# kspalaiologos/bzip3

Measured on AMD Instinct MI355X. Metric: MiB/s encode+decode round-trip, 8 MiB blocks, higher is better.
Workload: dtype u8

## Files before the change

bzip3_amd/__init__.py:

```python
import ctypes as C
import os

_HERE = os.path.dirname(os.path.abspath(__file__))
LIB_PATH = os.path.join(_HERE, "lib", "libbzip3.so")

BZ3_OK = 0
BZ3_ERR_OUT_OF_BOUNDS = -1
BZ3_ERR_BWT = -2
BZ3_ERR_CRC = -3
BZ3_ERR_MALFORMED_HEADER = -4
BZ3_ERR_TRUNCATED_DATA = -5
BZ3_ERR_DATA_TOO_BIG = -6
BZ3_ERR_INIT = -7
BZ3_ERR_DATA_SIZE_TOO_SMALL = -8

T_NAMES = ["crc", "rle", "lzp", "bwt", "cm", "copy", "_6", "_7"]

_lib = None


def _declare(L, strict=True):
    vp, i32, u32, sz = C.c_void_p, C.c_int32, C.c_uint32, C.c_size_t
    sig = {
        "bz3_version": (C.c_char_p, []),
# ... 23 lines not shown
        "bz3_hip_cm_variant_for": (C.c_int, [C.c_int, C.c_int, C.c_int]),
        "bz3_hip_set_lean_states": (C.c_int, [C.c_int]),
        "bz3_hip_release_cached_memory": (None, []),
        "bz3_hip_set_keep_workspace": (C.c_int, [C.c_int]),
        "bz3_hip_set_front_end_duo": (C.c_int, [C.c_int]),
        "bz3_hip_set_workspace_headroom": (None, [C.c_longlong]),
        "bz3_hip_workspace_headroom": (sz, []),
        "bz3_hip_debug_headroom_events": (C.c_uint, [C.c_int, C.POINTER(C.c_uint)]),
        "bz3_hip_debug_ring_contexts": (sz, [sz, sz, sz, sz, sz, sz, C.c_int, sz]),
        "bz3_hip_debug_arena_slack": (sz, [sz]),
        "bz3_hip_debug_cm_launches": (C.c_uint, [C.c_int]),
        "bz3_hip_debug_workspace_bytes": (sz, [sz, C.c_int]),
        "bz3_hip_debug_cached_bytes": (sz, [C.c_int]),
        "bz3_hip_encode_block_device": (i32, [vp, vp, i32]),
        "bz3_hip_decode_block_device": (i32, [vp, vp, sz, i32, i32]),
        "bz3_hip_encode_blocks_device": (None, [vp, vp, vp, i32]),
        "bz3_hip_decode_blocks_device": (None, [vp, vp, vp, vp, vp, i32]),
        "bz3_hip_compress_device": (C.c_int, [u32, vp, vp, sz, C.POINTER(sz)]),
        "bz3_hip_decompress_device": (C.c_int, [vp, vp, sz, C.POINTER(sz)]),
        "bz3_hip_frame_decoded_size_device": (C.c_int, [vp, sz, C.POINTER(sz)]),
        "bz3_hip_compress_device_many": (C.c_int, [u32, i32, C.POINTER(vp), C.POINTER(sz), C.POINTER(vp), C.POINTER(sz), C.POINTER(C.c_int)]),
        "bz3_hip_decompress_device_many": (C.c_int, [i32, C.POINTER(vp), C.POINTER(sz), C.POINTER(vp), C.POINTER(sz), C.POINTER(C.c_int)]),
        "bz3_hip_frame_decoded_sizes_device": (C.c_int, [i32, C.POINTER(vp), C.POINTER(sz), C.POINTER(sz), C.POINTER(C.c_int)]),
        "bz3_hip_debug_copy_segments": (i32, [vp, vp, C.POINTER(C.c_uint64), i32]),
        "bz3_hip_compress_device_planes": (C.c_int, [u32, u32, vp, vp, sz, C.POINTER(sz)]),
        "bz3_hip_decompress_device_planes": (C.c_int, [u32, vp, vp, sz, C.POINTER(sz)]),
        "bz3_hip_compress_device_planes_many": (C.c_int, [u32, i32, C.POINTER(u32), C.POINTER(vp), C.POINTER(sz), C.POINTER(vp), C.POINTER(sz), C.POINTER(C.c_int)]),
        "bz3_hip_decompress_device_planes_many": (C.c_int, [i32, C.POINTER(u32), C.POINTER(vp), C.POINTER(sz), C.POINTER(vp), C.POINTER(sz), C.POINTER(C.c_int)]),
        "bz3_hip_debug_planes": (i32, [vp, vp, C.POINTER(C.c_uint64), i32]),
        "bz3_hip_compress_device_delta": (C.c_int, [u32, u32, vp, vp, vp, sz, C.POINTER(sz)]),
        "bz3_hip_decompress_device_delta": (C.c_int, [u32, vp, vp, sz, vp, sz, C.POINTER(sz)]),
        "bz3_hip_compress_device_delta_many": (C.c_int, [u32, i32, C.POINTER(u32), C.POINTER(vp), C.POINTER(vp), C.POINTER(sz), C.POINTER(vp), C.POINTER(sz), C.POINTER(C.c_int)]),
        "bz3_hip_decompress_device_delta_many": (C.c_int, [i32, C.POINTER(u32), C.POINTER(vp), C.POINTER(sz), C.POINTER(vp), C.POINTER(sz), C.POINTER(vp), C.POINTER(sz), C.POINTER(C.c_int)]),
        "bz3_hip_crc32c_device": (C.c_int, [vp, sz, u32, C.POINTER(u32)]),
        "bz3_hip_crc32c_device_many": (C.c_int, [i32, C.POINTER(vp), C.POINTER(sz), C.POINTER(u32), C.POINTER(u32)]),
        "bz3_hip_debug_crc_launches": (C.c_uint, [C.c_int]),
        "bz3_hip_debug_delta": (i32, [vp, vp, vp, C.POINTER(C.c_uint64), i32]),
        "bz3_hip_decompress_device_range": (C.c_int, [u32, vp, sz, C.c_uint64, vp, sz, vp, C.POINTER(sz)]),
        "bz3_hip_decompress_device_range_many": (C.c_int, [i32, C.POINTER(u32), C.POINTER(vp), C.POINTER(sz), C.POINTER(C.c_uint64), C.POINTER(vp), C.POINTER(sz),
                                                           C.POINTER(vp), C.POINTER(sz), C.POINTER(C.c_int)]),
        "bz3_hip_debug_range": (i32, [vp, vp, vp, C.POINTER(C.c_uint64), i32]),
        "bz3_hip_last_timings": (None, [vp, C.POINTER(C.c_float)]),
        "bz3_hip_last_bwt_stats": (None, [vp, C.POINTER(i32), C.POINTER(i32), C.POINTER(C.c_uint64)]),
        "bz3_hip_stage_crc32c": (u32, [vp, sz, u32]),
        "bz3_hip_stage_mrle_encode": (i32, [vp, i32, vp]),
        "bz3_hip_stage_mrle_decode": (C.c_int, [vp, vp, i32, i32]),
        "bz3_hip_stage_lzp_encode": (i32, [vp, i32, vp]),
        "bz3_hip_stage_lzp_decode": (i32, [vp, i32, vp, i32]),
        "bz3_hip_stage_bwt": (i32, [vp, vp, i32]),
        "bz3_hip_stage_unbwt": (i32, [vp, vp, i32, i32]),
        "bz3_hip_stage_last_ms": (C.c_float, []),
        "bz3_hip_debug_sort_u32": (i32, [vp, u32, C.c_int, C.c_int, vp, vp]),
        "bz3_hip_debug_scan_u32": (i32, [vp, u32, vp]),
        "bz3_hip_debug_cu_masks": (i32, [C.c_int, C.c_int, vp, vp]),
        "bz3_hip_set_collect_window_us": (None, [C.c_int]),
        "bz3_hip_debug_collected_batches": (C.c_uint, [C.c_int, C.POINTER(C.c_uint)]),
        "bz3_hip_stage_cm_encode": (i32, [vp, i32, vp]),
        "bz3_hip_stage_cm_decode": (None, [vp, i32, vp, i32]),
        "bz3_hip_stage_cm_decode_many": (C.c_float, [vp, i32, vp, i32, i32, vp]),
        "bz3_hip_stage_cm_encode_many": (C.c_float, [vp, i32, vp, C.POINTER(i32), i32]),
        "bz3_hip_encode_stream": (C.c_int, [C.c_int, C.c_int, i32, i32]),
        "bz3_hip_decode_stream": (C.c_int, [C.c_int, C.c_int, i32]),
    }
    for name, (res, args) in sig.items():
        if not strict and not hasattr(L, name):
            continue
        fn = getattr(L, name)
        fn.restype = res
        fn.argtypes = args
    return L


EXPORTED_SYMBOLS = None


def _share_hip_runtime_with_torch():
    if os.environ.get("BZ3_HIP_SYSTEM_RUNTIME") == "1":
        return
    try:
        import importlib.util

        spec = importlib.util.find_spec("torch")
        if spec is None or not spec.origin:
            return
        cand = os.path.join(os.path.dirname(spec.origin), "lib", "libamdhip64.so")
        if os.path.exists(cand):
            C.CDLL(cand, mode=C.RTLD_GLOBAL)
    except Exception:
        pass


def load(path=None):
    global _lib
    if _lib is not None and path is None:
        return _lib
    if path is None:
        _share_hip_runtime_with_torch()
    p = path or LIB_PATH
    if not os.path.exists(p):
        raise RuntimeError(
            f"{p} is missing: the HIP extension has not been built (python -m bzip3_amd.build). "
            "bzip3_amd has no CPU or PyTorch fallback by design."
        )
    L = _declare(C.CDLL(p), strict=path is None)
    if path is None:
        _lib = L
# ... 844 lines not shown
```

bzip3_amd/csrc/api.hip:

```cpp
#include <atomic>
#include <chrono>
#include <condition_variable>
#include <cstdio>
#include <cstdlib>
#include <exception>
#include <mutex>
#include <new>
#include <stdexcept>
#include <thread>
#include <type_traits>
#include <vector>

#include "../../include/bz3_hip.h"
#include "frame.hpp"
#include "planes.hpp"
#include "prims.hpp"
#include "sort.hpp"
#include "stages.hpp"

using namespace bz3;

namespace {

constexpr s32 KiB65 = 65 * 1024;
// ... 3115 lines not shown
        bwt_inverse(d, (u32)n, (u32)idx, o, a, e.s);
        HIP_CHECK(hipStreamSynchronize(e.s));
        g_stage_ms.store(std::chrono::duration<float, std::milli>(std::chrono::steady_clock::now() - t0).count());
        e.down(out, o, (size_t)n);
        return 0;
    });
}

BZIP3_API int32_t bz3_hip_debug_cu_masks(int cus, int reserve, uint32_t * side, uint32_t * rest) {
    if (cus < 32 || cus > 1024 || reserve < 8 || !side || !rest) return -1;
    std::vector<uint32_t> a, b;
    DeviceCtx::cu_masks(cus, reserve, a, b);
    for (size_t k = 0; k < a.size(); k++) {
        side[k] = a[k];
        rest[k] = b[k];
    }
    return (int32_t)a.size();
}

BZIP3_API int32_t bz3_hip_debug_scan_u32(uint32_t * data, uint32_t n, uint32_t * total) {
    return stage_guard([&]() -> s32 {
        if (n == 0) return -1;
        StageEnv e;
        u32 * d = (u32 *)e.dev((size_t)n * 4 + 64, data, (size_t)n * 4);
        u32 * t = (u32 *)e.dev(64);
        Arena a = e.ctx->arena_for(scan_temp_words(n) * 4 + (1u << 20));
        exclusive_scan_u32(d, n, t, a, e.s);
        e.down(data, d, (size_t)n * 4);
        if (total) *total = e.word(t);
        return 0;
    });
}

BZIP3_API int32_t bz3_hip_debug_sort_u32(const uint32_t * keys, uint32_t n, int key_bits, int digit_bits, uint32_t * sorted_keys, uint32_t * sorted_index) {
    return stage_guard([&]() -> s32 {
        if ((digit_bits != 8 && digit_bits != 9) || key_bits < 1 || key_bits > 32 || n == 0) return -1;
        StageEnv e;
        u32 * k[2] = {(u32 *)e.dev((size_t)n * 4 + 64, keys, (size_t)n * 4), (u32 *)e.dev((size_t)n * 4 + 64)};
        u32 * v[2] = {(u32 *)e.dev((size_t)n * 4 + 64), (u32 *)e.dev((size_t)n * 4 + 64)};
        Arena a = e.ctx->arena_for(radix_temp_bytes(n, digit_bits) + (1u << 20));
        int cur = 0, passes = 0;
        for (int shift = 0; shift < key_bits; shift += digit_bits, passes++) {
            const u32 * vin = passes ? v[cur] : nullptr;
            if (digit_bits == 9) radix_pass_bits<u32, 9>(k[cur], k[cur ^ 1], vin, v[cur ^ 1], n, shift, 0xFFFFFFFFu, 0u, a, e.s);
            else radix_pass<u32>(k[cur], k[cur ^ 1], vin, v[cur ^ 1], n, shift, 0xFFFFFFFFu, 0u, a, e.s);
            cur ^= 1;
        }
        e.down(sorted_keys, k[cur], (size_t)n * 4);
        e.down(sorted_index, v[cur], (size_t)n * 4);
        return passes;
    });
}

extern "C++" template <class Job, class Launch>
void stage_cm_job(StageEnv & e, Job job, Launch && go) {
    const int variant = cm_variant_for(e.ctx, 1, std::is_same<Job, CmEncodeJob>::value);
    u32 * status = nullptr;
    if (cm_variant_has_rows(variant)) {
        job.spill = dev_addr(e.dev(CM_SPILL_BYTES));
        status = (u32 *)e.dev(64);
        HIP_CHECK(hipMemsetAsync(status, 0, 64, e.s));
        job.status = dev_addr(status);
        job.miss_base = cm_variant_is_test(variant) ? 64u : CM_MISS_BASE;
        job.miss_shift = cm_variant_is_test(variant) ? 3u : CM_MISS_SHIFT;
    }
    Job * d_job = (Job *)e.dev(sizeof job, &job, sizeof job);
    go(d_job, 1u, e.s, variant);
    if (cm_variant_has_rows(variant) && e.word(status) != 0u) {
        g_cm_given_up.fetch_add(1u);
        go(d_job, 1u, e.s, (int)CM_VARIANT_FULL);
    }
}

BZIP3_API int32_t bz3_hip_stage_cm_encode(const uint8_t * in, int32_t n, uint8_t * out) {
    return stage_guard([&]() -> s32 {
        StageEnv e;
        u8 * d = e.dev((size_t)n + 64, in, (size_t)n);
        u8 * o = e.dev(bz3_bound((size_t)n) + 64);
        u32 * w = (u32 *)e.dev(64);
        const char * dbg = getenv("BZ3_CM_DEBUG");
        CmEncodeJob job{dev_addr(d), dev_addr(o), dev_addr(w), (u32)n, dbg ? (u32)atoi(dbg) : 0u};
        const char * tg = getenv("BZ3_CM_TEST_GAP");
        u8 * side = nullptr;
        if (tg) {
            const size_t g = (size_t)atol(tg);
            const char * ts = getenv("BZ3_CM_TEST_SIDE");
            const size_t side_cap = ts ? (size_t)atol(ts) : CM_SIDE_BYTES;
            u8 * both = e.dev(g + (size_t)n + 64);
            HIP_CHECK(hipMemcpy(both + g, d, (size_t)n, hipMemcpyDeviceToDevice));
            side = e.dev(side_cap + 64);
            o = both;
            job.in = dev_addr(both + g);
            job.out = dev_addr(both);
            job.gap = (u32)g;
            job.side = dev_addr(side);
            job.side_cap = (u32)side_cap;
        }
        stage_cm_job(e, job, [](const CmEncodeJob * j, u32 nj, hipStream_t st, int variant) { cm_encode_batch(j, nj, st, variant); });
        const u32 coded = e.word(w), sw = e.word(w + 1);
        if (coded == 0xFFFFFFFFu) return -1;
        const u32 head = (tg && sw < coded) ? sw : coded;
        e.down(out, o, (size_t)head);
        if (head < coded) e.down(out + head, side, (size_t)(coded - head));
        return (s32)coded;
    });
}
// ... 123 lines not shown
```

bzip3_amd/csrc/bwt.hip:

```cpp
#include <atomic>
#include <vector>

#include "prims.hpp"
#include "sort.hpp"
#include "stages.hpp"

namespace bz3 {

constexpr int BW_BLOCK = 256;
constexpr u32 V_HEAD = 0x80000000u;
constexpr u32 V_MASK = 0x3FFFFFFFu;

__global__ void __launch_bounds__(256) k_bwt_outside(const u32 * __restrict__ hist, u32 keep, u32 * __restrict__ out) {
    __shared__ u32 h[256];
    __shared__ u32 red[256 / WAVE + 1];
    const u32 c = threadIdx.x;
    h[c] = hist[c];
    __syncthreads();
    const u32 mine = h[c];
    u32 rank = 0;
    for (u32 k = 0; k < 256u; k++) rank += (h[k] > mine || (h[k] == mine && k < c)) ? 1u : 0u;
    const u32 tot = block_sum<256>(rank >= keep ? mine : 0u, red);
    if (c == 0) *out = tot;
}
// ... 1232 lines not shown
                st_g[out] = rank[j];
                out++;
            }
        }
    }
    __syncthreads();
    for (u32 idx = threadIdx.x; idx < all; idx += BW_BLOCK) {
        vals_out[tile_off + idx] = st_v[idx];
        slots_out[tile_off + idx] = st_s[idx];
        grp_out[tile_off + idx] = st_g[idx];
    }
}

__global__ void __launch_bounds__(BW_BLOCK) k_bwt_doubling_keys_grp(const u32 * __restrict__ vals, const u32 * __restrict__ grp, const u32 * __restrict__ isa, u32 m,
                                                                   u32 n, u32 h, u64 * __restrict__ keys) {
    const u32 k = blockIdx.x * BW_BLOCK + threadIdx.x;
    if (k >= m) return;
    const u32 s = vals[k];
    const u64 j = (u64)s + h;
    const u32 lo = (j < n) ? isa[j] + h : (n - 1u - s);
    keys[k] = ((u64)grp[k] << 32) | lo;
}

constexpr int IS_ITEMS = 8;
__global__ void __launch_bounds__(BW_BLOCK) k_isa_scatter(const u32 * __restrict__ suf, const u32 * __restrict__ rank, u32 n, u32 tiles, u32 * __restrict__ isa) {
    const u32 per = (tiles + 7u) / 8u;
    const u32 tile = (blockIdx.x & 7u) * per + (blockIdx.x >> 3);
    if (tile >= tiles) return;
    const u64 base = (u64)tile * (BW_BLOCK * IS_ITEMS) + threadIdx.x;
    u32 x[IS_ITEMS], r[IS_ITEMS];
#pragma unroll
    for (int k = 0; k < IS_ITEMS; k++) {
        const u64 i = base + (u64)k * BW_BLOCK;
        x[k] = suf[i < n ? i : (u64)n - 1];
        r[k] = rank[i < n ? i : (u64)n - 1];
    }
#pragma unroll
    for (int k = 0; k < IS_ITEMS; k++)
        if (base + (u64)k * BW_BLOCK < n) isa[x[k] & V_MASK] = r[k];
}

static int bits_for(u64 x) {
    int b = 0;
    while (x) { b++; x >>= 1; }
    return b ? b : 1;
}

size_t bwt_workspace_bytes(u64 n) {
    return n * (16 + 8 + 1 + 11 + 4 + 8 + 4 + 4 + 4) + n / 8 + radix_temp_bytes(n) + scan_temp_words(n) * 4 + (1u << 20) + 16384 + VLC_WORK_BYTES;
}

template <typename K>
static int sort_iota(const K * kin, K * k0, K * k1, u32 * v0, u32 * v1, u64 n, int bit_lo, int bit_hi, Arena & tmp, hipStream_t s, BwtStats & st) {
    radix_pass<K>(kin, k1, (const u32 *)nullptr, v1, n, bit_lo, 0xFFFFFFFFu, 0u, tmp, s);
    int cur = 1;
    K * kk[2] = {k0, k1};
    u32 * vv[2] = {v0, v1};
    st.radix_passes++;
    for (int shift = bit_lo + 8; shift < bit_hi; shift += 8) {
        radix_pass<K>(kk[cur], kk[cur ^ 1], (const u32 *)vv[cur], vv[cur ^ 1], n, shift, 0xFFFFFFFFu, 0u, tmp, s);
        cur ^= 1;
        st.radix_passes++;
    }
    return cur;
}

struct BwtSwitches {
    bool trace;
    int big_rounds_default;
    std::atomic<int> big_rounds;
};
static BwtSwitches & bwt_switches() {
    static BwtSwitches sw{getenv("BZ3_BWT_TRACE") != nullptr, getenv("BZ3_BWT_BIG_ROUNDS") ? atoi(getenv("BZ3_BWT_BIG_ROUNDS")) : 1,
                          {getenv("BZ3_BWT_BIG_ROUNDS") ? atoi(getenv("BZ3_BWT_BIG_ROUNDS")) : 1}};
    return sw;
}
void bwt_set_big_rounds(int k) { bwt_switches().big_rounds.store(k < 0 ? bwt_switches().big_rounds_default : k); }
struct BwtGrids {
    u32 wide, tail;
};
static BwtGrids bwt_grids(u32 n) {
    static const BwtGrids forced = [] {
        BwtGrids g{0, 0};
        if (const char * e = getenv("BZ3_BWT_GRIDS")) (void)sscanf(e, "%u,%u", &g.wide, &g.tail);
        return g;
    }();
    if (forced.wide && forced.tail) return forced;
    const u32 tail = n / (64u * 4u), wide = n / (64u * 4u * 16u);
    return BwtGrids{wide < 8u ? 8u : wide, tail < 32u ? 32u : tail};
}

__global__ void k_bwt_set_word(u32 * p, u32 v) { *p = v; }

s32 bwt_forward(const u8 * d_in, u32 n, u8 * d_out, Arena & tmp, hipStream_t s, BwtStats * stats, u32 * d_idx, u32 * d_outside) {
    if (d_outside && n < 2) HIP_CHECK(hipMemsetAsync(d_outside, 0, 4, s));
    if (n == 0) {
        if (d_idx) launch(k_bwt_set_word, dim3(1), dim3(1), 0, s, d_idx, 0u);
        return 0;
    }
    if (n == 1) {
        HIP_CHECK(hipMemcpyAsync(d_out, d_in, 1, hipMemcpyDeviceToDevice, s));
        if (d_idx) {
            launch(k_bwt_set_word, dim3(1), dim3(1), 0, s, d_idx, 1u);
            return 0;
        }
        HIP_CHECK(hipStreamSynchronize(s));
        return 1;
    }
    if (n > V_MASK) throw HipError{hipErrorUnknown, "block too large for the suffix sorter", __FILE__, __LINE__};
    const size_t mk = tmp.mark();
    u64 * key[2] = {tmp.take<u64>(n), tmp.take<u64>(n)};
    u32 * val[2] = {tmp.take<u32>(n), tmp.take<u32>(n)};
    u8 * pb = tmp.take<u8>(n);
    const u32 tiles = (u32)(((u64)n + TR_S - 1) / TR_S);
    u32 * tile_last = tmp.take<u32>(tiles + 1);
    u32 * carry = tmp.take<u32>(tiles + 1);
    const u32 sp_groups = (tiles + SP_GROUP - 1) / SP_GROUP;
    u32 * group_max = tmp.take<u32>(sp_groups + 1);
    u32 * group_carry = tmp.take<u32>(sp_groups + 1);
    u8 * dirty = tmp.take<u8>(tiles + 2);
    u32 * hbits = tmp.take<u32>(((size_t)n + 63) / 64 * 2 + (size_t)TR_S / 32 + 8);
    u32 * d_words = tmp.take<u32>(16);
    u32 * d_vlc = tmp.take<u32>(256);
    u32 * d_hist = tmp.take<u32>(256);
    BwtStats st;

    auto grid = [](u64 m) { return dim3((u32)((m + BW_BLOCK - 1) / BW_BLOCK)); };

    HIP_CHECK(hipMemsetAsync(d_hist, 0, 256 * sizeof(u32), s));
    HIP_CHECK(hipMemsetAsync(d_words, 0, 16 * sizeof(u32), s));
    HIP_CHECK(hipMemsetAsync(d_words + 5, 0xFF, sizeof(u32), s));
    launch(k_bwt_sym_hist, grid(((u64)n + 63) / 64), dim3(BW_BLOCK), 0, s, d_in, n, d_hist);
    if (d_outside) launch(k_bwt_outside, dim3(1), dim3(256), 0, s, (const u32 *)d_hist, (u32)BWT_ROUTE_KEEP, d_outside);
    {
        const size_t vm = tmp.mark();
        vlc_build_device(d_hist, d_vlc, tmp, s);
        tmp.release(vm);
    }

    launch(k_bwt_vlc_keys, grid(((u64)n + 7) / 8), dim3(BW_BLOCK), 0, s, d_in, n, (const u32 *)d_vlc, key[0]);
    const int cur = sort_iota<u64>(key[0], key[0], key[1], val[0], val[1], n, 8, 64, tmp, s, st);
    st.sorted_elements += n;
    st.rounds++;
    u32 * V = val[cur];
    launch(k_bwt_heads, dim3(tiles), dim3(BW_BLOCK), 0, s, (const u64 *)key[cur], V, pb, n, tile_last, hbits, d_words);
    launch(k_bwt_spine_a, dim3(sp_groups), dim3(SP_BLOCK), 0, s, (const u32 *)tile_last, tiles, carry, group_max);
    launch(k_bwt_spine_b, dim3(1), dim3(1024), 0, s, (const u32 *)group_max, sp_groups, group_carry);

    const u32 big_cap = n / 4;
    char * scratch = reinterpret_cast<char *>(key[0]);
    (void)scratch;
    u32 * big_slot = reinterpret_cast<u32 *>(key[0]);
    u32 * big_hp = big_slot + big_cap;
    u32 * bord[2] = {big_hp + big_cap, big_hp + 2 * (size_t)big_cap};
    u32 * bgk[2] = {bord[1] + big_cap, bord[1] + 2 * (size_t)big_cap};
    u32 * gv = bgk[1] + big_cap;
    u32 * ghp = gv + big_cap;
    u64 * bkey0 = key[1];
    u64 * bkey[2] = {bkey0 + big_cap, bkey0 + 2 * (size_t)big_cap};
    u64 * gkey = bkey0 + 3 * (size_t)big_cap;
    u8 * gpb = reinterpret_cast<u8 *>(val[cur ^ 1]);
    const u32 tail_cap = n;
    u32 * tail_v = tmp.take<u32>(tail_cap);
    u32 * tail_slot = tmp.take<u32>(tail_cap);
    u16 * tail_d = tmp.take<u16>(tail_cap);
    u8 * tail_pb = tmp.take<u8>(tail_cap);
    const u32 mid_cap = n / 64 + 16;
    u32 * mid_slot = tmp.take<u32>(mid_cap);
    u16 * mid_size = tmp.take<u16>(mid_cap);
    u32 g = 7;
    bool deep = false;
    u32 h_words[16];
    const BwtGrids grids = bwt_grids(n);
    for (int pass = 0;; pass++) {
        launch(k_bwt_route, dim3((tiles + RT_WAVES - 1) / RT_WAVES), dim3(RT_WAVES * WAVE), 0, s, n, (const u32 *)V, (const u8 *)pb, (const u32 *)hbits,
               (const u32 *)carry, (const u32 *)group_carry, (const u8 *)(pass ? dirty : nullptr), big_slot, big_hp, big_cap, mid_slot, mid_size, mid_cap, tail_v, tail_slot,
               tail_d, tail_pb, tail_cap, d_words);
        launch(k_bwt_wide, dim3(grids.wide), dim3(WR_WAVES * WAVE), 0, s, d_in, n, V, pb, (const u32 *)d_vlc, (const u32 *)mid_slot, (const u16 *)mid_size, mid_cap, tail_v,
               tail_slot, tail_d, tail_pb, tail_cap, d_words, (u32)pass + 1u);
        launch(k_bwt_tail, dim3(grids.tail), dim3(WAVE), 0, s, d_in, n, V, pb, (const u32 *)d_vlc, (const u32 *)tail_v, (const u32 *)tail_slot, (const u16 *)tail_d,
               (const u8 *)tail_pb, d_words, (u32)pass + 1u);
        HIP_CHECK(hipMemcpyAsync(h_words, d_words, sizeof h_words, hipMemcpyDeviceToHost, s));
        HIP_CHECK(hipStreamSynchronize(s));
        const u32 nb = h_words[0];
        if (bwt_switches().trace) fprintf(stderr, "[bwt] n %u pass %d depth %u: %u suffixes in groups > %d, %u groups through the wide kernel, %u suffixes through the tail kernel, %u given up, overflow %u\n", n, pass, g, nb, TR_G, h_words[8], h_words[4], h_words[1], h_words[3]);
        if (nb == 0) {
            deep = h_words[1] != 0;
            break;
        }
        const int max_big = bwt_switches().big_rounds.load();
        if (h_words[3] || pass >= max_big || nb > n / 4) {
            deep = true;
            break;
        }
        st.rounds++;
        st.sorted_elements += nb;
        launch(k_big_keys, grid(nb), dim3(BW_BLOCK), 0, s, d_in, n, (const u32 *)V, (const u32 *)d_vlc, (const u32 *)big_slot, nb, (u32)pass + 1u, bkey0);
        int c = sort_iota<u64>(bkey0, bkey[0], bkey[1], bord[0], bord[1], nb, 0, 57, tmp, s, st);
        u32 * order = bord[c];
        u32 * ofree = bord[c ^ 1];
        launch(k_big_order_keys, grid(nb), dim3(BW_BLOCK), 0, s, (const u32 *)order, (const u32 *)big_hp, nb, bgk[0]);
        {
            const int hb = bits_for(n);
            u32 * oo[2] = {order, ofree};
            const int c2 = radix_sort_pairs<u32>(bgk[0], bgk[1], oo[0], oo[1], nb, 0, hb, tmp, s);
            st.radix_passes += (hb + 7) / 8;
            order = oo[c2];
            ofree = oo[c2 ^ 1];
        }
        launch(k_big_gather, grid(nb), dim3(BW_BLOCK), 0, s, (const u32 *)order, (const u32 *)big_slot, (const u32 *)big_hp, (const u64 *)bkey0, (const u32 *)V,
               (const u8 *)pb, nb, gv, gpb, gkey, ghp);
        {
            const int hb = bits_for(n);
            HIP_CHECK(hipMemcpyAsync(bgk[0], big_slot, (size_t)nb * 4, hipMemcpyDeviceToDevice, s));
            u32 * oo[2] = {order, ofree};
            const int c3 = radix_sort_pairs<u32>(bgk[0], bgk[1], oo[0], oo[1], nb, 0, hb, tmp, s);
            st.radix_passes += (hb + 7) / 8;
            HIP_CHECK(hipMemsetAsync(dirty, 0, tiles + 2, s));
            launch(k_big_apply, grid(nb), dim3(BW_BLOCK), 0, s, (const u32 *)bgk[c3], (const u32 *)gv, (const u8 *)gpb, (const u64 *)gkey, (const u32 *)ghp, nb, V, pb,
                   dirty, d_words);
        }
        g += 7;
        HIP_CHECK(hipMemsetAsync(d_words, 0, sizeof(u32), s));
        HIP_CHECK(hipMemsetAsync(d_words + 4, 0, sizeof(u32), s));
        HIP_CHECK(hipMemsetAsync(d_words + 5, 0xFF, sizeof(u32), s));
        HIP_CHECK(hipMemsetAsync(d_words + 8, 0, sizeof(u32), s));
        launch(k_bwt_reduce_heads, dim3(tiles), dim3(BW_BLOCK), 0, s, (const u32 *)V, n, tile_last, hbits);
        launch(k_bwt_spine_a, dim3(sp_groups), dim3(SP_BLOCK), 0, s, (const u32 *)tile_last, tiles, carry, group_max);
    launch(k_bwt_spine_b, dim3(1), dim3(1024), 0, s, (const u32 *)group_max, sp_groups, group_carry);
    }

    u32 idx = 0;
    if (!deep) {
        launch(k_bwt_finish, grid(n), dim3(BW_BLOCK), 0, s, d_in, (const u8 *)pb, n, (const u32 *)(d_words + 2), d_out, d_words + 7);
    } else {
        u32 * sa = V;
        u32 * isa = tmp.take<u32>(n);
        u32 * slot[2] = {tmp.take<u32>(n), tmp.take<u32>(n)};
        u32 * grp = tmp.take<u32>(n);
        u32 * vv[2] = {val[cur ^ 1], tmp.take<u32>(n)};
        const u32 max_tiles = (u32)(((u64)n + BG_TILE - 1) / BG_TILE);
        u32 * tile_head = tmp.take<u32>(2 * (size_t)max_tiles + 16);
        u32 * tile_keep = tile_head + max_tiles + 8;
        u32 m = n, h = g < 7u + 5u * (u32)TL_CAP ? g : 7u + 5u * (u32)TL_CAP;
        if (bwt_switches().trace) fprintf(stderr, "[bwt] n %u deep path from depth %u\n", n, h);
        {
            u32 * rk = reinterpret_cast<u32 *>(key[0]);
            u32 * kb = rk + n;
            u32 * rb = reinterpret_cast<u32 *>(key[1]);
            const u32 tl = (u32)(((u64)m + BG_TILE - 1) / BG_TILE);
            launch(k_bg_reduce<true>, dim3(tl), dim3(BW_BLOCK), 0, s, (const u64 *)nullptr, (const u32 *)V, m, tile_head, tile_keep);
            launch(k_bg_spine, dim3(1), dim3(BG_SPINE), 0, s, tile_head, tile_keep, tl, d_words + 6);
            launch(k_bg_apply<true, false>, dim3(tl), dim3(BW_BLOCK), 0, s, (const u64 *)nullptr, (const u32 *)V, (const u32 *)nullptr, m, (const u32 *)tile_head,
                   (const u32 *)tile_keep, sa, isa, vv[0], slot[0], grp, d_in, pb, rk);
            const int nbits = bits_for((u64)n - 1);
            const int shift = nbits > 8 ? nbits - 8 : 0;
            radix_pass<u32>((const u32 *)V, kb, (const u32 *)rk, rb, n, shift, 0xFFFFFFFFu, 0u, tmp, s);
            st.radix_passes++;
            const u32 itiles = (u32)(((u64)n + BW_BLOCK * IS_ITEMS - 1) / (BW_BLOCK * IS_ITEMS));
            launch(k_isa_scatter, dim3(8u * ((itiles + 7u) / 8u)), dim3(BW_BLOCK), 0, s, (const u32 *)kb, (const u32 *)rb, n, itiles, isa);
        }
        int scur = 0;
        u32 * vact = vv[0], * vfree = vv[1];
        for (;;) {
            u32 m_next = 0;
            HIP_CHECK(hipMemcpyAsync(&m_next, d_words + 6, 4, hipMemcpyDeviceToHost, s));
            HIP_CHECK(hipStreamSynchronize(s));
            if (m_next == 0) break;
            m = m_next;
            st.rounds++;
            if (bwt_switches().trace) fprintf(stderr, "[bwt] n %u doubling round at depth %u: %u active suffixes\n", n, h, m);
            launch(k_bwt_doubling_keys_grp, grid(m), dim3(BW_BLOCK), 0, s, (const u32 *)vact, (const u32 *)grp, (const u32 *)isa, m, n, h, key[0]);
            u32 * pv[2] = {vact, vfree};
            const int lo_bits = bits_for((u64)n + h);
            const int hi_bits = bits_for(n);
            int c = radix_sort_pairs<u64>(key[0], key[1], pv[0], pv[1], m, 0, lo_bits, tmp, s);
            c ^= radix_sort_pairs<u64>(key[c], key[c ^ 1], pv[c], pv[c ^ 1], m, 32, 32 + hi_bits, tmp, s);
            u32 * vsorted = pv[c];
            vfree = pv[c ^ 1];
// ... 28 lines not shown
```

bzip3_amd/csrc/sort.hip:

```cpp
#include "prims.hpp"
#include "sort.hpp"

namespace bz3 {

constexpr int SC_BLOCK = 256;
constexpr int SC_ITEMS = 8;
constexpr int SC_TILE = SC_BLOCK * SC_ITEMS;

__device__ __forceinline__ void scan_load_items(const u32 * __restrict__ data, u64 n, u64 base, u32 (&v)[SC_ITEMS]) {
    static_assert(SC_ITEMS == 8, "two uint4 per thread");
    if (base + SC_ITEMS <= n && (reinterpret_cast<uintptr_t>(data) & 15u) == 0) {
        const uint4 a = *reinterpret_cast<const uint4 *>(data + base);
        const uint4 b = *reinterpret_cast<const uint4 *>(data + base + 4);
        v[0] = a.x; v[1] = a.y; v[2] = a.z; v[3] = a.w;
        v[4] = b.x; v[5] = b.y; v[6] = b.z; v[7] = b.w;
    } else {
        const u64 last = n - 1;
#pragma unroll
        for (int k = 0; k < SC_ITEMS; k++) v[k] = data[base + k < n ? base + k : last];
#pragma unroll
        for (int k = 0; k < SC_ITEMS; k++) v[k] = base + k < n ? v[k] : 0u;
    }
}

__global__ void __launch_bounds__(SC_BLOCK) k_scan_reduce(const u32 * __restrict__ data, u64 n, u32 * __restrict__ sums) {
    __shared__ u32 lds[SC_BLOCK / WAVE + 1];
    const u64 base = (u64)blockIdx.x * SC_TILE + (u64)threadIdx.x * SC_ITEMS;
    u32 v[SC_ITEMS];
    scan_load_items(data, n, base, v);
    u32 acc = 0;
#pragma unroll
    for (int k = 0; k < SC_ITEMS; k++) acc += v[k];
    u32 tot = block_sum<SC_BLOCK>(acc, lds);
    if (threadIdx.x == 0) sums[blockIdx.x] = tot;
}

__global__ void __launch_bounds__(SC_BLOCK) k_scan_apply(u32 * __restrict__ data, u64 n, const u32 * __restrict__ sums,
                                                         u32 * __restrict__ total_out) {
    __shared__ u32 lds[SC_BLOCK / WAVE + 1];
    const u64 base = (u64)blockIdx.x * SC_TILE + (u64)threadIdx.x * SC_ITEMS;
    u32 v[SC_ITEMS];
    scan_load_items(data, n, base, v);
    u32 acc = 0;
#pragma unroll
    for (int k = 0; k < SC_ITEMS; k++) acc += v[k];
    u32 tot;
    u32 pre = block_excl_add<SC_BLOCK>(acc, lds, tot);
    if (sums) pre += sums[blockIdx.x];
    if (base + SC_ITEMS <= n && (reinterpret_cast<uintptr_t>(data) & 15u) == 0) {
        uint4 a, b;
        a.x = pre; a.y = a.x + v[0]; a.z = a.y + v[1]; a.w = a.z + v[2];
        b.x = a.w + v[3]; b.y = b.x + v[4]; b.z = b.y + v[5]; b.w = b.z + v[6];
// ... 254 lines not shown
    }
    __syncthreads();
    const u64 left = n - tile_base;
    const u32 count = left < (u64)RS_TILE ? (u32)left : (u32)RS_TILE;
#pragma unroll
    for (int q = 0; q < RS_ROUNDS; q++) {
        const u32 j = (u32)q * RS_BLOCK + threadIdx.x;
        if (j < count) {
            const K k = skey[j];
            const u32 pos = gdelta[rs_digit<K, BITS>(k, shift)] + j;
            if (WKEYS) kout[pos] = k;
            vout[pos] = sval[j];
        }
    }
}

constexpr u32 RS_RAW_TILES = 128;

template <typename K, int BITS>
void radix_pass_bits(const K * kin, K * kout, const u32 * vin, u32 * vout, u64 n, int shift, u32 iota_split, u32 out_base, Arena & tmp,
                     hipStream_t s) {
    if (n == 0) return;
    constexpr int RADIX = 1 << BITS;
    const u32 tiles = (u32)((n + RS_TILE - 1) / RS_TILE);
    size_t m = tmp.mark();
    u32 * hist = tmp.take<u32>((size_t)tiles * RADIX);
    const u32 xcd = 1u;
    const dim3 sgrid(rs_grid(tiles, xcd != 0u));
    launch(k_rs_hist<K, BITS>, sgrid, dim3(RS_BLOCK), 0, s, kin, n, shift, hist, tiles, xcd);
    static const bool no_raw = getenv("BZ3_RS_NO_RAW") != nullptr;
    const bool raw = tiles <= RS_RAW_TILES && !no_raw;
    if (!raw) exclusive_scan_u32(hist, (u64)tiles * RADIX, nullptr, tmp, s);
    const bool iota = vin == nullptr, wkeys = kout != nullptr;
#define BZ3_RS_LAUNCH(I, W, R) \
    launch(k_rs_scatter<K, I, W, BITS, R>, sgrid, dim3(RS_BLOCK), 0, s, kin, kout, vin, vout, n, shift, (const u32 *)hist, tiles, iota_split, out_base, xcd)
#define BZ3_RS_DISPATCH(R)                                   \
    do {                                                     \
        if (iota && wkeys) BZ3_RS_LAUNCH(true, true, R);     \
        else if (iota) BZ3_RS_LAUNCH(true, false, R);        \
        else if (wkeys) BZ3_RS_LAUNCH(false, true, R);       \
        else BZ3_RS_LAUNCH(false, false, R);                 \
    } while (0)
    if (raw) BZ3_RS_DISPATCH(true);
    else BZ3_RS_DISPATCH(false);
#undef BZ3_RS_DISPATCH
#undef BZ3_RS_LAUNCH
    tmp.release(m);
}

void radix_hist_bits9(const u32 * keys, u64 n, int shift, u32 * hist, u32 tiles, hipStream_t s) {
    launch(k_rs_hist<u32, 9>, dim3(rs_grid(tiles, true)), dim3(RS_BLOCK), 0, s, keys, n, shift, hist, tiles, 1u);
}

template <typename K>
void radix_pass(const K * kin, K * kout, const u32 * vin, u32 * vout, u64 n, int shift, u32 iota_split, u32 out_base, Arena & tmp,
                hipStream_t s) {
    radix_pass_bits<K, 8>(kin, kout, vin, vout, n, shift, iota_split, out_base, tmp, s);
}

template <typename K>
int radix_sort_pairs(K * k0, K * k1, u32 * v0, u32 * v1, u64 n, int bit_lo, int bit_hi, Arena & tmp, hipStream_t s) {
    int cur = 0;
    for (int shift = bit_lo; shift < bit_hi; shift += 8) {
        if (cur == 0)
            radix_pass<K>(k0, k1, v0, v1, n, shift, 0xFFFFFFFFu, 0u, tmp, s);
        else
            radix_pass<K>(k1, k0, v1, v0, n, shift, 0xFFFFFFFFu, 0u, tmp, s);
        cur ^= 1;
    }
    return cur;
}

template void radix_pass<u8>(const u8 *, u8 *, const u32 *, u32 *, u64, int, u32, u32, Arena &, hipStream_t);
template void radix_pass<u32>(const u32 *, u32 *, const u32 *, u32 *, u64, int, u32, u32, Arena &, hipStream_t);
template void radix_pass<u64>(const u64 *, u64 *, const u32 *, u32 *, u64, int, u32, u32, Arena &, hipStream_t);
template void radix_pass_bits<u32, 9>(const u32 *, u32 *, const u32 *, u32 *, u64, int, u32, u32, Arena &, hipStream_t);
template int radix_sort_pairs<u32>(u32 *, u32 *, u32 *, u32 *, u64, int, int, Arena &, hipStream_t);
template int radix_sort_pairs<u64>(u64 *, u64 *, u32 *, u32 *, u64, int, int, Arena &, hipStream_t);

}
```

bzip3_amd/csrc/sort.hpp:

```cpp
#pragma once
#include "hipx.hpp"

namespace bz3 {

struct Arena {
    char * base = nullptr;
    size_t cap = 0, used = 0;
    template <typename T>
    T * take(size_t count) {
        size_t bytes = (count * sizeof(T) + 255) & ~(size_t)255;
        if (used + bytes > cap) throw HipError{hipErrorUnknown, "device workspace exhausted", __FILE__, __LINE__};
        T * p = reinterpret_cast<T *>(base + used);
        used += bytes;
        return p;
    }
    size_t mark() const { return used; }
    void release(size_t m) { used = m; }
};

constexpr int RS_TILE = 4096;
constexpr int RS_BLOCK = 256;
constexpr int RS_RADIX = 256;

inline size_t scan_temp_words(u64 n) {
    size_t w = 0;
    while (n > 2048) {
        n = (n + 2047) / 2048;
        w += ((n + 63) & ~(u64)63);
    }
    return w + 64;
}
inline size_t radix_temp_bytes(u64 n, int bits = 8) {
    u64 tiles = (n + RS_TILE - 1) / RS_TILE;
    u64 hist = tiles << bits;
    return (hist + scan_temp_words(hist) + 256) * 4 + 4096;
}

void exclusive_scan_u32(u32 * d_data, u64 n, u32 * d_total, Arena & tmp, hipStream_t s);

template <typename K>
void radix_pass(const K * kin, K * kout, const u32 * vin, u32 * vout, u64 n, int shift, u32 iota_split, u32 out_base,
                Arena & tmp, hipStream_t s);

template <typename K, int BITS>
void radix_pass_bits(const K * kin, K * kout, const u32 * vin, u32 * vout, u64 n, int shift, u32 iota_split, u32 out_base,
                     Arena & tmp, hipStream_t s);

void radix_hist_bits9(const u32 * keys, u64 n, int shift, u32 * hist, u32 tiles, hipStream_t s);

template <typename K>
int radix_sort_pairs(K * k0, K * k1, u32 * v0, u32 * v1, u64 n, int bit_lo, int bit_hi, Arena & tmp, hipStream_t s);

}
```

include/bz3_hip.h:

```cpp
#ifndef BZ3_HIP_H
#define BZ3_HIP_H
#include <stddef.h>
#include <stdint.h>
#include "libbz3.h"
#define BZ3_HIP 1

#ifdef __cplusplus
extern "C" {
#endif

BZIP3_API int bz3_hip_device_count(void);
BZIP3_API int bz3_hip_bind_device(int device);
BZIP3_API int bz3_hip_state_device(struct bz3_state * state);

BZIP3_API int bz3_hip_set_cm_mode(int mode);
BZIP3_API void bz3_hip_debug_bwt_big_rounds(int k);
BZIP3_API unsigned bz3_hip_cm_blocks_given_up(void);
BZIP3_API unsigned bz3_hip_cm_blocks_routed_full(void);

BZIP3_API int bz3_hip_cm_variant_for(int device, int blocks, int encode);

BZIP3_API int bz3_hip_debug_peak_concurrent_groups(int reset);

BZIP3_API int bz3_hip_debug_front_end_ring(void);
// ... 36 lines not shown
BZIP3_API int bz3_hip_compress_device_planes_many(uint32_t block_size, int32_t n, const uint32_t elem_sizes[], const void * const ins[],
                                                  const size_t in_sizes[], void * const outs[], size_t out_sizes[], int rcs[]);
BZIP3_API int bz3_hip_decompress_device_planes_many(int32_t n, const uint32_t elem_sizes[], const void * const ins[],
                                                    const size_t in_sizes[], void * const outs[], size_t out_sizes[], int rcs[]);
BZIP3_API int32_t bz3_hip_debug_planes(const void * src, void * dst, const uint64_t * segs, int32_t n);

BZIP3_API int bz3_hip_compress_device_delta(uint32_t block_size, uint32_t elem_size, const void * in, const void * base, void * out,
                                            size_t in_size, size_t * out_size);
BZIP3_API int bz3_hip_decompress_device_delta(uint32_t elem_size, const void * in, const void * base, size_t base_size, void * out,
                                              size_t in_size, size_t * out_size);
BZIP3_API int bz3_hip_compress_device_delta_many(uint32_t block_size, int32_t n, const uint32_t elem_sizes[], const void * const ins[],
                                                 const void * const bases[], const size_t in_sizes[], void * const outs[],
                                                 size_t out_sizes[], int rcs[]);
BZIP3_API int bz3_hip_decompress_device_delta_many(int32_t n, const uint32_t elem_sizes[], const void * const ins[],
                                                   const size_t in_sizes[], const void * const bases[], const size_t base_sizes[],
                                                   void * const outs[], size_t out_sizes[], int rcs[]);
BZIP3_API int bz3_hip_crc32c_device(const void * p, size_t n, uint32_t init, uint32_t * crc);
BZIP3_API int bz3_hip_crc32c_device_many(int32_t n, const void * const * ptrs, const size_t * sizes, const uint32_t * inits, uint32_t * crcs);
BZIP3_API unsigned bz3_hip_debug_crc_launches(int reset);
BZIP3_API int32_t bz3_hip_debug_delta(const void * src, const void * base, void * dst, const uint64_t * segs, int32_t n);

BZIP3_API int bz3_hip_decompress_device_range(uint32_t elem_size, const void * in, size_t in_size, uint64_t offset, const void * base,
                                              size_t base_size, void * out, size_t * out_size);
BZIP3_API int bz3_hip_decompress_device_range_many(int32_t n, const uint32_t elem_sizes[], const void * const ins[], const size_t in_sizes[],
                                                   const uint64_t offsets[], const void * const bases[], const size_t base_sizes[],
                                                   void * const outs[], size_t out_sizes[], int rcs[]);
BZIP3_API int32_t bz3_hip_debug_range(const void * src, const void * base, void * dst, const uint64_t * segs, int32_t n);

enum {
    BZ3_HIP_T_CRC = 0,
    BZ3_HIP_T_RLE = 1,
    BZ3_HIP_T_LZP = 2,
    BZ3_HIP_T_BWT = 3,
    BZ3_HIP_T_CM = 4,
    BZ3_HIP_T_COPY = 5,
    BZ3_HIP_T_COUNT = 8
};
BZIP3_API void bz3_hip_last_timings(struct bz3_state * state, float ms[BZ3_HIP_T_COUNT]);
BZIP3_API void bz3_hip_last_bwt_stats(struct bz3_state * state, int32_t * rounds, int32_t * radix_passes, uint64_t * sorted_elements);

BZIP3_API void bz3_hip_set_collect_window_us(int us);
BZIP3_API unsigned bz3_hip_debug_collected_batches(int reset, unsigned * largest);

BZIP3_API uint32_t bz3_hip_stage_crc32c(const uint8_t * data, size_t n, uint32_t init);
BZIP3_API int32_t bz3_hip_stage_mrle_encode(const uint8_t * in, int32_t n, uint8_t * out);
BZIP3_API int bz3_hip_stage_mrle_decode(const uint8_t * in, uint8_t * out, int32_t outlen, int32_t maxin);
BZIP3_API int32_t bz3_hip_stage_lzp_encode(const uint8_t * in, int32_t n, uint8_t * out);
BZIP3_API int32_t bz3_hip_stage_lzp_decode(const uint8_t * in, int32_t n, uint8_t * out, int32_t max);
BZIP3_API int32_t bz3_hip_stage_bwt(const uint8_t * in, uint8_t * out, int32_t n);
BZIP3_API int32_t bz3_hip_stage_unbwt(const uint8_t * in, uint8_t * out, int32_t n, int32_t idx);
BZIP3_API int32_t bz3_hip_debug_cu_masks(int cus, int reserve, uint32_t * side, uint32_t * rest);
BZIP3_API int32_t bz3_hip_debug_scan_u32(uint32_t * data, uint32_t n, uint32_t * total);
BZIP3_API int32_t bz3_hip_debug_sort_u32(const uint32_t * keys, uint32_t n, int key_bits, int digit_bits, uint32_t * sorted_keys, uint32_t * sorted_index);
BZIP3_API float bz3_hip_stage_last_ms(void);
BZIP3_API int32_t bz3_hip_stage_cm_encode(const uint8_t * in, int32_t n, uint8_t * out);
BZIP3_API void bz3_hip_stage_cm_decode(const uint8_t * in, int32_t in_size, uint8_t * out, int32_t n);

#define BZ3_HIP_ERR_IO (-100)
BZIP3_API int bz3_hip_encode_stream(int in_fd, int out_fd, int32_t block_size, int32_t blocks_per_batch);
BZIP3_API int bz3_hip_decode_stream(int in_fd, int out_fd, int32_t blocks_per_batch);

BZIP3_API float bz3_hip_stage_cm_decode_many(const uint8_t * in, int32_t in_size, uint8_t * out, int32_t n, int32_t copies, uint64_t * counters);

BZIP3_API float bz3_hip_stage_cm_encode_many(const uint8_t * in, int32_t n, uint8_t * out, int32_t * coded, int32_t copies);

#ifdef __cplusplus
}
#endif
#endif
```

Baseline: 634.5.

## Add single-block multi-pass radix sort for small inputs and fuse BWT resets

Adds a single-workgroup radix sort kernel that runs all passes for inputs up to a size threshold inside one launch, keeping intermediate passes in LDS when small enough. radix_pass, radix_sort_pairs and sort_iota route small sorts through it, cutting per-pass multi-kernel launch overhead for the many small group sorts in the BWT. Separately, several hipMemsetAsync calls in the BWT rounds are replaced by small reset kernels. The risk is that one block handles up to 4096 keys serially, and the ballot-based ranking must preserve stability.

Result: no change. 636.5, median of 6 (+0.3%).

```diff
diff --git a/bzip3_amd/__init__.py b/bzip3_amd/__init__.py
--- a/bzip3_amd/__init__.py
+++ b/bzip3_amd/__init__.py
@@ -99,6 +99,8 @@
         "bz3_hip_stage_last_ms": (C.c_float, []),
         "bz3_hip_debug_sort_u32": (i32, [vp, u32, C.c_int, C.c_int, vp, vp]),
         "bz3_hip_debug_scan_u32": (i32, [vp, u32, vp]),
+        "bz3_hip_debug_rs_small_max": (u32, [C.c_int64]),
+        "bz3_hip_debug_sort_pairs": (i32, [vp, vp, u32, C.c_int, C.c_int, C.c_int, vp, vp, C.c_int, C.POINTER(C.c_float)]),
         "bz3_hip_debug_cu_masks": (i32, [C.c_int, C.c_int, vp, vp]),
         "bz3_hip_set_collect_window_us": (None, [C.c_int]),
         "bz3_hip_debug_collected_batches": (C.c_uint, [C.c_int, C.POINTER(C.c_uint)]),
diff --git a/bzip3_amd/csrc/api.hip b/bzip3_amd/csrc/api.hip
--- a/bzip3_amd/csrc/api.hip
+++ b/bzip3_amd/csrc/api.hip
@@ -3191,6 +3191,42 @@
     });
 }
 
+BZIP3_API uint32_t bz3_hip_debug_rs_small_max(int64_t keys) {
+    const u32 before = radix_small_max();
+    radix_set_small_max(keys);
+    return before;
+}
+
+BZIP3_API int32_t bz3_hip_debug_sort_pairs(const void * keys, const uint32_t * values, uint32_t n, int key_bytes, int bit_lo, int bit_hi, void * sorted_keys,
+                                           uint32_t * sorted_values, int reps, float * ms) {
+    return stage_guard([&]() -> s32 {
+        if ((key_bytes != 4 && key_bytes != 8) || bit_lo < 0 || bit_hi > 8 * key_bytes || bit_lo > bit_hi || n == 0 || reps < 1) return -1;
+        StageEnv e;
+        const size_t kb = (size_t)n * (size_t)key_bytes, vb = (size_t)n * 4;
+        u8 * src_k = e.dev(kb + 64, keys, kb);
+        u8 * src_v = e.dev(vb + 64, values, vb);
+        u8 * k[2] = {e.dev(kb + 64), e.dev(kb + 64)};
+        u32 * v[2] = {(u32 *)e.dev(vb + 64), (u32 *)e.dev(vb + 64)};
+        Arena a = e.ctx->arena_for(radix_temp_bytes(n) + (1u << 20));
+        int cur = 0;
+        double total = 0;
+        for (int r = 0; r < reps; r++) {
+            HIP_CHECK(hipMemcpyAsync(k[0], src_k, kb, hipMemcpyDeviceToDevice, e.s));
+            HIP_CHECK(hipMemcpyAsync(v[0], src_v, vb, hipMemcpyDeviceToDevice, e.s));
+            HIP_CHECK(hipStreamSynchronize(e.s));
+            const auto t0 = std::chrono::steady_clock::now();
+            if (key_bytes == 8) cur = radix_sort_pairs<u64>((u64 *)k[0], (u64 *)k[1], v[0], v[1], n, bit_lo, bit_hi, a, e.s);
+            else cur = radix_sort_pairs<u32>((u32 *)k[0], (u32 *)k[1], v[0], v[1], n, bit_lo, bit_hi, a, e.s);
+            HIP_CHECK(hipStreamSynchronize(e.s));
+            total += std::chrono::duration<double, std::milli>(std::chrono::steady_clock::now() - t0).count();
+        }
+        if (ms) *ms = (float)(total / reps);
+        e.down(sorted_keys, k[cur], kb);
+        e.down(sorted_values, v[cur], vb);
+        return cur;
+    });
+}
+
 extern "C++" template <class Job, class Launch>
 void stage_cm_job(StageEnv & e, Job job, Launch && go) {
     const int variant = cm_variant_for(e.ctx, 1, std::is_same<Job, CmEncodeJob>::value);
diff --git a/bzip3_amd/csrc/bwt.hip b/bzip3_amd/csrc/bwt.hip
--- a/bzip3_amd/csrc/bwt.hip
+++ b/bzip3_amd/csrc/bwt.hip
@@ -1308,6 +1308,13 @@
 
 template <typename K>
 static int sort_iota(const K * kin, K * k0, K * k1, u32 * v0, u32 * v1, u64 n, int bit_lo, int bit_hi, Arena & tmp, hipStream_t s, BwtStats & st) {
+    {
+        const int npasses = 1 + (bit_hi > bit_lo + 8 ? (bit_hi - bit_lo - 8 + 7) / 8 : 0);
+        if (radix_sort_small<K>(kin, (const u32 *)nullptr, k1, v1, k0, v0, n, bit_lo, npasses, 0xFFFFFFFFu, 0u, true, s)) {
+            st.radix_passes += npasses;
+            return npasses & 1;
+        }
+    }
     radix_pass<K>(kin, k1, (const u32 *)nullptr, v1, n, bit_lo, 0xFFFFFFFFu, 0u, tmp, s);
     int cur = 1;
     K * kk[2] = {k0, k1};
@@ -1347,6 +1354,21 @@
 }
 
 __global__ void k_bwt_set_word(u32 * p, u32 v) { *p = v; }
+
+__global__ void __launch_bounds__(256) k_bwt_reset(u32 * __restrict__ hist, u32 * __restrict__ words) {
+    hist[threadIdx.x] = 0u;
+    if (threadIdx.x < 16) words[threadIdx.x] = threadIdx.x == 5 ? 0xFFFFFFFFu : 0u;
+}
+__global__ void __launch_bounds__(BW_BLOCK) k_bwt_round_reset(u8 * __restrict__ dirty, u32 count, u32 * __restrict__ words) {
+    const u32 i = blockIdx.x * BW_BLOCK + threadIdx.x;
+    if (i < count) dirty[i] = 0;
+    if (i == 0) {
+        words[0] = 0u;
+        words[4] = 0u;
+        words[5] = 0xFFFFFFFFu;
+        words[8] = 0u;
+    }
+}
 
 s32 bwt_forward(const u8 * d_in, u32 n, u8 * d_out, Arena & tmp, hipStream_t s, BwtStats * stats, u32 * d_idx, u32 * d_outside) {
     if (d_outside && n < 2) HIP_CHECK(hipMemsetAsync(d_outside, 0, 4, s));
@@ -1383,9 +1405,7 @@
 
     auto grid = [](u64 m) { return dim3((u32)((m + BW_BLOCK - 1) / BW_BLOCK)); };
 
-    HIP_CHECK(hipMemsetAsync(d_hist, 0, 256 * sizeof(u32), s));
-    HIP_CHECK(hipMemsetAsync(d_words, 0, 16 * sizeof(u32), s));
-    HIP_CHECK(hipMemsetAsync(d_words + 5, 0xFF, sizeof(u32), s));
+    launch(k_bwt_reset, dim3(1), dim3(256), 0, s, d_hist, d_words);
     launch(k_bwt_sym_hist, grid(((u64)n + 63) / 64), dim3(BW_BLOCK), 0, s, d_in, n, d_hist);
     if (d_outside) launch(k_bwt_outside, dim3(1), dim3(256), 0, s, (const u32 *)d_hist, (u32)BWT_ROUTE_KEEP, d_outside);
     {
@@ -1472,15 +1492,11 @@
             u32 * oo[2] = {order, ofree};
             const int c3 = radix_sort_pairs<u32>(bgk[0], bgk[1], oo[0], oo[1], nb, 0, hb, tmp, s);
             st.radix_passes += (hb + 7) / 8;
-            HIP_CHECK(hipMemsetAsync(dirty, 0, tiles + 2, s));
+            launch(k_bwt_round_reset, grid((u64)tiles + 2), dim3(BW_BLOCK), 0, s, dirty, tiles + 2, d_words);
             launch(k_big_apply, grid(nb), dim3(BW_BLOCK), 0, s, (const u32 *)bgk[c3], (const u32 *)gv, (const u8 *)gpb, (const u64 *)gkey, (const u32 *)ghp, nb, V, pb,
                    dirty, d_words);
         }
         g += 7;
-        HIP_CHECK(hipMemsetAsync(d_words, 0, sizeof(u32), s));
-        HIP_CHECK(hipMemsetAsync(d_words + 4, 0, sizeof(u32), s));
-        HIP_CHECK(hipMemsetAsync(d_words + 5, 0xFF, sizeof(u32), s));
-        HIP_CHECK(hipMemsetAsync(d_words + 8, 0, sizeof(u32), s));
         launch(k_bwt_reduce_heads, dim3(tiles), dim3(BW_BLOCK), 0, s, (const u32 *)V, n, tile_last, hbits);
         launch(k_bwt_spine_a, dim3(sp_groups), dim3(SP_BLOCK), 0, s, (const u32 *)tile_last, tiles, carry, group_max);
     launch(k_bwt_spine_b, dim3(1), dim3(1024), 0, s, (const u32 *)group_max, sp_groups, group_carry);
diff --git a/bzip3_amd/csrc/sort.hip b/bzip3_amd/csrc/sort.hip
--- a/bzip3_amd/csrc/sort.hip
+++ b/bzip3_amd/csrc/sort.hip
@@ -1,3 +1,5 @@
+#include <atomic>
+
 #include "prims.hpp"
 #include "sort.hpp"
 
@@ -358,14 +360,137 @@
     launch(k_rs_hist<u32, 9>, dim3(rs_grid(tiles, true)), dim3(RS_BLOCK), 0, s, keys, n, shift, hist, tiles, 1u);
 }
 
+constexpr int RSS_BLOCK = 1024;
+constexpr int RSS_WAVES = RSS_BLOCK / WAVE;
+constexpr int RSS_UNROLL = 8;
+constexpr u32 RS_SMALL_LDS = 4096;
+
+template <typename K, bool INLDS>
+__global__ void __launch_bounds__(RSS_BLOCK) k_rs_small(const K * kin, const u32 * vin, K * ka, u32 * va, K * kb, u32 * vb, u32 n, int shift0,
+                                                          int npasses, u32 iota_split, u32 out_base, u32 wkeys) {
+    constexpr u32 NL = INLDS ? RS_SMALL_LDS : 1u;
+    __shared__ u32 cnt[RSS_WAVES][RS_RADIX];
+    __shared__ u32 scan_lds[RSS_WAVES + 1];
+    __shared__ K skey[2][NL];
+    __shared__ u32 sval[2][NL];
+    const int w = wave_id(), l = lane_id();
+    const u64 lt = lanemask_lt();
+    const u32 span = (n + RSS_BLOCK - 1) / RSS_BLOCK * WAVE;
+    const u32 wbeg = (u32)w * span;
+    const u32 last = n - 1;
+    const K * ksrc = kin;
+    const u32 * vsrc = vin;
+    for (int p = 0; p < npasses; p++) {
+        const int shift = shift0 + 8 * p;
+        const bool fin = p == npasses - 1;
+        K * kdst = (INLDS && !fin) ? skey[p & 1] : ((p & 1) ? kb : ka);
+        u32 * vdst = (INLDS && !fin) ? sval[p & 1] : ((p & 1) ? vb : va);
+        const u32 base = fin ? out_base : 0u;
+        const bool wk = fin ? wkeys != 0u : true;
+#pragma unroll
+        for (int k = 0; k < RSS_WAVES * RS_RADIX / RSS_BLOCK; k++) (&cnt[0][0])[k * RSS_BLOCK + threadIdx.x] = 0;
+        __syncthreads();
+        for (u32 r0 = 0; r0 < span; r0 += RSS_UNROLL * WAVE) {
+            K key[RSS_UNROLL];
+#pragma unroll
+            for (int r = 0; r < RSS_UNROLL; r++) {
+                const u32 i = wbeg + r0 + (u32)r * WAVE + l;
+                key[r] = ksrc[i < n ? i : last];
+            }
+#pragma unroll
+            for (int r = 0; r < RSS_UNROLL; r++) {
+                const u32 o = r0 + (u32)r * WAVE + l;
+                if (o < span && wbeg + o < n) atomicAdd(&cnt[w][rs_digit<K, 8>(key[r], shift)], 1u);
+            }
+        }
+        __syncthreads();
+        {
+            u32 run = 0;
+            if (threadIdx.x < RS_RADIX) {
+#pragma unroll
+                for (int k = 0; k < RSS_WAVES; k++) {
+                    const u32 c = cnt[k][threadIdx.x];
+                    cnt[k][threadIdx.x] = run;
+                    run += c;
+                }
+            }
+            u32 total;
+            const u32 start = block_excl_add<RSS_BLOCK>(run, scan_lds, total);
+            if (threadIdx.x < RS_RADIX) {
+#pragma unroll
+                for (int k = 0; k < RSS_WAVES; k++) cnt[k][threadIdx.x] += start + base;
+            }
+        }
+        __syncthreads();
+        for (u32 r0 = 0; r0 < span; r0 += RSS_UNROLL * WAVE) {
+            K key[RSS_UNROLL];
+            u32 val[RSS_UNROLL];
+#pragma unroll
+            for (int r = 0; r < RSS_UNROLL; r++) {
+                const u32 i = wbeg + r0 + (u32)r * WAVE + l;
+                key[r] = ksrc[i < n ? i : last];
+                val[r] = vsrc ? vsrc[i < n ? i : last] : i + (i >= iota_split ? 1u : 0u);
+            }
+#pragma unroll
+            for (int r = 0; r < RSS_UNROLL; r++) {
+                const u32 o = r0 + (u32)r * WAVE + l;
+                const bool valid = o < span && wbeg + o < n;
+                const u32 d = rs_digit<K, 8>(key[r], shift);
+                u64 peers = __ballot(valid);
+#pragma unroll
+                for (int b = 0; b < 8; b++) {
+                    const bool bit = (d >> b) & 1u;
+                    const u64 bal = __ballot(bit);
+                    peers &= bit ? bal : ~bal;
+                }
+                const u32 below = (u32)__popcll(peers & lt);
+                const u32 pre = valid ? cnt[w][d] : 0u;
+                wave_sync();
+                if (valid && below == 0) cnt[w][d] = pre + (u32)__popcll(peers);
+                wave_sync();
+                if (valid) {
+                    const u32 pos = pre + below;
+                    if (wk) kdst[pos] = key[r];
+                    vdst[pos] = val[r];
+                }
+            }
+        }
+        __threadfence_block();
+        __syncthreads();
+        ksrc = kdst;
+        vsrc = vdst;
+    }
+}
+
+static std::atomic<u32> g_rs_small_max{[] {
+    const char * e = getenv("BZ3_RS_SMALL_MAX");
+    return e ? (u32)strtoul(e, nullptr, 10) : RS_SMALL_MAX;
+}()};
+u32 radix_small_max() { return g_rs_small_max.load(std::memory_order_relaxed); }
+void radix_set_small_max(s64 keys) { g_rs_small_max.store(keys < 0 ? RS_SMALL_MAX : (u32)keys); }
+
+template <typename K>
+bool radix_sort_small(const K * kin, const u32 * vin, K * ka, u32 * va, K * kb, u32 * vb, u64 n, int shift0, int npasses, u32 iota_split, u32 out_base,
+                      bool wkeys, hipStream_t s) {
+    if (n == 0 || npasses <= 0 || n > radix_small_max()) return false;
+    if (n <= RS_SMALL_LDS && npasses > 1)
+        launch(k_rs_small<K, true>, dim3(1), dim3(RSS_BLOCK), 0, s, kin, vin, ka, va, kb, vb, (u32)n, shift0, npasses, iota_split, out_base, wkeys ? 1u : 0u);
+    else
+        launch(k_rs_small<K, false>, dim3(1), dim3(RSS_BLOCK), 0, s, kin, vin, ka, va, kb, vb, (u32)n, shift0, npasses, iota_split, out_base, wkeys ? 1u : 0u);
+    return true;
+}
+
 template <typename K>
 void radix_pass(const K * kin, K * kout, const u32 * vin, u32 * vout, u64 n, int shift, u32 iota_split, u32 out_base, Arena & tmp,
                 hipStream_t s) {
+    if (radix_sort_small<K>(kin, vin, kout, vout, (K *)nullptr, (u32 *)nullptr, n, shift, 1, iota_split, out_base, kout != nullptr, s)) return;
     radix_pass_bits<K, 8>(kin, kout, vin, vout, n, shift, iota_split, out_base, tmp, s);
 }
 
 template <typename K>
 int radix_sort_pairs(K * k0, K * k1, u32 * v0, u32 * v1, u64 n, int bit_lo, int bit_hi, Arena & tmp, hipStream_t s) {
+    const int npasses = bit_hi > bit_lo ? (bit_hi - bit_lo + 7) / 8 : 0;
+    if (radix_sort_small<K>(k0, v0, k1, v1, k0, v0, n, bit_lo, npasses, 0xFFFFFFFFu, 0u, true, s)) return npasses & 1;
     int cur = 0;
     for (int shift = bit_lo; shift < bit_hi; shift += 8) {
         if (cur == 0)
@@ -381,6 +506,8 @@
 template void radix_pass<u32>(const u32 *, u32 *, const u32 *, u32 *, u64, int, u32, u32, Arena &, hipStream_t);
 template void radix_pass<u64>(const u64 *, u64 *, const u32 *, u32 *, u64, int, u32, u32, Arena &, hipStream_t);
 template void radix_pass_bits<u32, 9>(const u32 *, u32 *, const u32 *, u32 *, u64, int, u32, u32, Arena &, hipStream_t);
+template bool radix_sort_small<u32>(const u32 *, const u32 *, u32 *, u32 *, u32 *, u32 *, u64, int, int, u32, u32, bool, hipStream_t);
+template bool radix_sort_small<u64>(const u64 *, const u32 *, u64 *, u32 *, u64 *, u32 *, u64, int, int, u32, u32, bool, hipStream_t);
 template int radix_sort_pairs<u32>(u32 *, u32 *, u32 *, u32 *, u64, int, int, Arena &, hipStream_t);
 template int radix_sort_pairs<u64>(u64 *, u64 *, u32 *, u32 *, u64, int, int, Arena &, hipStream_t);
 
diff --git a/bzip3_amd/csrc/sort.hpp b/bzip3_amd/csrc/sort.hpp
--- a/bzip3_amd/csrc/sort.hpp
+++ b/bzip3_amd/csrc/sort.hpp
@@ -48,6 +48,13 @@
 
 void radix_hist_bits9(const u32 * keys, u64 n, int shift, u32 * hist, u32 tiles, hipStream_t s);
 
+constexpr u32 RS_SMALL_MAX = 4096;
+u32 radix_small_max();
+void radix_set_small_max(s64 keys);
+template <typename K>
+bool radix_sort_small(const K * kin, const u32 * vin, K * ka, u32 * va, K * kb, u32 * vb, u64 n, int shift0, int npasses, u32 iota_split, u32 out_base,
+                      bool wkeys, hipStream_t s);
+
 template <typename K>
 int radix_sort_pairs(K * k0, K * k1, u32 * v0, u32 * v1, u64 n, int bit_lo, int bit_hi, Arena & tmp, hipStream_t s);
 
diff --git a/include/bz3_hip.h b/include/bz3_hip.h
--- a/include/bz3_hip.h
+++ b/include/bz3_hip.h
@@ -112,6 +112,9 @@
 BZIP3_API int32_t bz3_hip_debug_cu_masks(int cus, int reserve, uint32_t * side, uint32_t * rest);
 BZIP3_API int32_t bz3_hip_debug_scan_u32(uint32_t * data, uint32_t n, uint32_t * total);
 BZIP3_API int32_t bz3_hip_debug_sort_u32(const uint32_t * keys, uint32_t n, int key_bits, int digit_bits, uint32_t * sorted_keys, uint32_t * sorted_index);
+BZIP3_API uint32_t bz3_hip_debug_rs_small_max(int64_t keys);
+BZIP3_API int32_t bz3_hip_debug_sort_pairs(const void * keys, const uint32_t * values, uint32_t n, int key_bytes, int bit_lo, int bit_hi, void * sorted_keys,
+                                           uint32_t * sorted_values, int reps, float * ms);
 BZIP3_API float bz3_hip_stage_last_ms(void);
 BZIP3_API int32_t bz3_hip_stage_cm_encode(const uint8_t * in, int32_t n, uint8_t * out);
 BZIP3_API void bz3_hip_stage_cm_decode(const uint8_t * in, int32_t in_size, uint8_t * out, int32_t n);
```
